# JohannesErnst/WeaSAL

Hardware: AMD Instinct MI355X
Metric: points/sec fwd+bwd KPFCNN on DALES spheres; achieved HBM GB/s on KPConv gather (higher is better)
Workload: dtype f32; 1 GPU; DALES_PseudoLabel KP-FCNN, in_radius=10m, 50k pts/sphere, batch=8, fp32, step = GPU pyramid + fwd + loss + bwd + SGD; contrast_loss term included (trainer_PseudoLabel.py:204-208); pyramid of the next batch overlapped on a second stream; parallelism=dp1, dist_world_size=1, allreduce_bytes=0

## Files before the change

include/weasal_hip.h:

```cpp
#ifndef WEASAL_HIP_H
#define WEASAL_HIP_H

#include <stdint.h>

#ifdef __cplusplus
extern "C" {
#endif

typedef enum {
    WS_OK = 0,
    WS_ERR_INVALID = 1,
    WS_ERR_UNSUPPORTED = 2,
    WS_ERR_HIP = 3,
    WS_ERR_EMPTY = 4,
    WS_ERR_CAPACITY = 5
} ws_status;

enum { WS_INFLUENCE_LINEAR = 0, WS_INFLUENCE_CONSTANT = 1, WS_INFLUENCE_GAUSSIAN = 2 };
enum { WS_AGGREGATION_SUM = 0, WS_AGGREGATION_CLOSEST = 1 };

const char* ws_last_error(void);
int64_t ws_launch_count(void);
const char* ws_version(void);
int ws_device_count(void);
// ... 96 lines not shown
                                     int32_t* d_max_count, void* stream);
int ws_radius_neighbors_nearest_async(ws_neighbors_ws* ws, const float* queries, int64_t nq, const float* supports,
                                      int64_t ns, const int32_t* h_q_lens, const int32_t* h_s_lens, int32_t nb,
                                      float radius, int32_t* out_i32, int64_t* out_i64, int32_t* d_any, void* stream);
int ws_radius_neighbors_order(const ws_neighbors_ws* ws, int32_t* out_order, void* stream);
const int32_t* ws_radius_neighbors_counts(const ws_neighbors_ws* ws);

int ws_radius_neighbors_set_key_last(ws_neighbors_ws* ws, uint64_t* d_key_last);
int ws_radius_neighbors_reuse_grid(ws_neighbors_ws* ws, int32_t on);
int ws_radius_neighbors_grid_info(const ws_neighbors_ws* ws, int32_t* nb, int64_t* cells, int64_t* ns, int64_t* blob_bytes);
int ws_radius_neighbors_grid_export(const ws_neighbors_ws* ws, void* blob, void* stream);
int ws_kpconv_gather_bwd_x_grid(const float* s_pts, int64_t ns, const void* grid_blob, int32_t nb, int64_t cells,
                                const uint64_t* key_last, float radius, const float* dwf, int32_t ci,
                                const float* kernel_points, int32_t k, const float* deformed_kp, const float* modulations,
                                float extent, int32_t influence, int32_t aggregation, const int32_t* order, float* dx,
                                int32_t* overflow, void* stream);

int ws_kpconv_gather_bwd_x_gated(const float* q_pts, int64_t nq, const float* s_pts, int64_t ns,
                                 const int64_t* inds, int32_t h, const int32_t* t_offsets, const int32_t* t_pairs,
                                 const float* dwf, int32_t ci, const float* kernel_points, int32_t k,
                                 const float* deformed_kp, const float* modulations, float extent,
                                 int32_t influence, int32_t aggregation, const int32_t* order, const float* gate_y,
                                 float gate_slope, float* dx, void* stream);
int ws_kpconv_gather_bwd_x_grid_gated(const float* s_pts, int64_t ns, const void* grid_blob, int32_t nb, int64_t cells,
                                      const uint64_t* key_last, float radius, const float* dwf, int32_t ci,
                                      const float* kernel_points, int32_t k, const float* deformed_kp, const float* modulations,
                                      float extent, int32_t influence, int32_t aggregation, const int32_t* order,
                                      const float* gate_y, float gate_slope, const int64_t* rows, int32_t rows_h, float* dx,
                                      int32_t* overflow, void* stream);

enum { WS_ORDER_REFERENCE = 0, WS_ORDER_FIRST_SEEN = 1 };
typedef struct ws_subsample_ws ws_subsample_ws;
int ws_subsample_ws_create(ws_subsample_ws** ws);
void ws_subsample_ws_destroy(ws_subsample_ws* ws);
int ws_grid_subsample_plan(ws_subsample_ws* ws, const float* points, int64_t n,
                           const int32_t* h_lens, int32_t nb, float dl, int32_t max_p,
                           int32_t order_mode, int32_t* h_out_lens, int64_t* h_m, void* stream);
int ws_grid_subsample_fill(ws_subsample_ws* ws,
                           const float* features, int32_t fd,
                           const int32_t* labels, int32_t ld,
                           float* out_points, float* out_features, int32_t* out_labels,
                           uint64_t* out_keys,
                           int32_t* out_counts,
                           void* stream);

int ws_rotate_clouds(const float* points, int64_t n, const int32_t* lens , int32_t nb,
// ... 304 lines not shown
```

weasal_amd/_lib.py:

```python
import ctypes as C
import os

_HERE = os.path.dirname(os.path.abspath(__file__))
LIB_PATH = os.path.join(_HERE, "libweasal_hip.so")

_vp = C.c_void_p
_i32 = C.c_int32
_i64 = C.c_int64
_f32 = C.c_float

SIGNATURES = {
    "ws_last_error": (C.c_char_p, []),
    "ws_version": (C.c_char_p, []),
    "ws_device_count": (C.c_int, []),
    "ws_kpconv_gather_fwd": (C.c_int, [_vp, _i64, _vp, _i64, _vp, _i32, _vp, _i32, _vp, _i32, _vp, _vp,
                                      _f32, _i32, _i32, _vp, _vp, _vp, _vp]),
    "ws_kpconv_gather_bwd_x": (C.c_int, [_vp, _i64, _vp, _i64, _vp, _i32, _vp, _vp, _vp, _i32, _vp, _i32,
                                        _vp, _vp, _f32, _i32, _i32, _vp, _vp, _vp]),
    "ws_kpconv_gather_bwd_geom": (C.c_int, [_vp, _i64, _vp, _i64, _vp, _i32, _vp, _i32, _vp, _vp, _i32,
                                           _vp, _vp, _vp, _f32, _i32, _i32, _vp, _vp, _vp]),
    "ws_transpose_scratch_bytes": (_i64, [_i64, _i32, _i64]),
    "ws_transpose_build": (C.c_int, [_vp, _i64, _i32, _i64, _vp, _vp, _vp, _vp]),
    "ws_max_pool_fwd": (C.c_int, [_vp, _i64, _i32, _vp, _i64, _i32, _vp, _vp, _vp]),
    "ws_max_pool_bwd": (C.c_int, [_vp, _vp, _i64, _i32, _i32, _vp, _vp, _i64, _vp, _vp]),
# ... 67 lines not shown
                                                   C.c_float, _i32, _i32, _vp, _vp, _vp, _vp]),
    "ws_max_pool_fwd_bf16": (C.c_int, [_vp, _i64, _i32, _vp, _i64, _i32, _vp, _vp, _vp]),
    "ws_max_pool_bwd_bf16": (C.c_int, [_vp, _vp, _i64, _i32, _i32, _vp, _vp, _i64, _vp, _vp]),
    "ws_closest_pool_fwd_bf16": (C.c_int, [_vp, _i64, _i32, _vp, _i64, _i32, _vp, _vp]),
    "ws_closest_pool_bwd_bf16": (C.c_int, [_vp, _i64, _i32, _i32, _vp, _vp, _i64, _vp, _vp]),
    "ws_gemm_xbt_bf16": (C.c_int, [_vp, _i64, _i32, _i64, _vp, _i32, _i64, _vp, _vp, _i64, _i32, _f32, _vp, _i64, _i32, _vp]),
    "ws_gemm_xty_bf16": (C.c_int, [_vp, _i64, _i32, _i64, _vp, _i32, _i64, _vp, _vp, _vp]),
    "ws_act_bwd_colsum_bf16_scratch_bytes": (_i64, [_i64, _i32]),
    "ws_act_bwd_colsum_bf16": (C.c_int, [_vp, _i32, _i64, _i32, _i64, _vp, _i64, C.c_float, _vp, _i64, _vp, _vp, _vp]),
    "ws_kpblock_fwd_scratch_bytes": (_i64, [_vp]),
    "ws_kpblock_bwd_scratch_bytes": (_i64, [_vp]),
    "ws_kpblock_fwd": (C.c_int, [_vp, _vp, _i64, _vp]),
    "ws_kpblock_bwd": (C.c_int, [_vp, _vp, _i64, _vp]),
    "ws_upunary_fwd_scratch_bytes": (_i64, [_vp]),
    "ws_upunary_bwd_scratch_bytes": (_i64, [_vp]),
    "ws_upunary_fwd": (C.c_int, [_vp, _vp, _i64, _vp]),
    "ws_upunary_bwd": (C.c_int, [_vp, _vp, _i64, _vp]),
    "ws_gemm_xb_epilogue_strided": (C.c_int, [_vp, _i64, _i32, _i64, _vp, _i64, _i64, _i32, _vp, _vp, _i64, _i32, _f32, _vp, _i64,
                                              _vp, _i64, _vp]),
    "ws_gemm_xb_gated_strided": (C.c_int, [_vp, _i64, _i32, _i64, _vp, _i64, _i64, _i32, _vp, _vp, _i64, _i32, _f32, _vp, _i64, _f32,
                                           _vp, _i64, _f32, _vp, _i64, _vp, _i64, _vp]),
    "ws_kpconv_gather_bwd_x_gated": (C.c_int, [_vp, _i64, _vp, _i64, _vp, _i32, _vp, _vp, _vp, _i32, _vp, _i32,
                                              _vp, _vp, _f32, _i32, _i32, _vp, _vp, _f32, _vp, _vp]),
    "ws_kpconv_gather_bwd_x_grid_gated": (C.c_int, [_vp, _i64, _vp, _i32, _i64, _vp, C.c_float, _vp, _i32, _vp, _i32, _vp, _vp,
                                                    C.c_float, _i32, _i32, _vp, _vp, _f32, _vp, _i32, _vp, _vp, _vp]),
    "ws_vote_update": (C.c_int, [_vp, _i64, _i32, _vp, _f32, _vp, _vp, _i64, _f32, _vp]),
    "ws_project_confusion": (C.c_int, [_vp, _i32, _vp, _i64, _vp, _vp, _i32, _vp, _vp]),
    "ws_potentials_scratch_bytes": (_i64, [_i64]),
    "ws_potentials_update": (C.c_int, [_vp, _i64, _vp, C.c_double, _vp, _vp, _vp, _vp, _vp]),
    "ws_al_point_scores": (C.c_int, [_vp, _i64, _i32, _vp, _vp, _vp, _vp, _vp]),
    "ws_al_anchor_scores": (C.c_int, [_vp, _vp, _i64, _vp, _vp, _i64, _i64, _vp, _i32, _vp, _vp]),
    "ws_topk_scratch_bytes": (_i64, [_i64, _i64]),
    "ws_topk_select": (C.c_int, [_vp, _i64, _vp, _i64, _i64, _vp, _vp, _vp]),
    "ws_weak_mask": (C.c_int, [_vp, _i64, _i32, _vp, _vp, _i64, _vp, _i64, _vp, _i64, _vp, _vp]),
    "ws_refine_labels": (C.c_int, [_vp, _vp, _i64, _i32, _vp, _vp, _i64, C.c_double, _i32, _vp, _vp, _i32, _vp, _vp]),
    "ws_anchor_bounds": (C.c_int, [_vp, _i64, _vp, _vp]),
    "ws_anchor_scratch_bytes": (_i64, [_i64]),
    "ws_anchor_members_plan": (C.c_int, [_vp, _vp, _i64, _i32, _vp, _i64, C.c_double, _vp, _vp, _vp, _vp, _vp, _vp, _vp, _vp, _vp,
                                        _vp, _vp]),
    "ws_anchor_members_fill": (C.c_int, [_vp, _i64, _vp, _i64, C.c_double, _vp, _vp, _vp, _vp, _vp, _vp, _vp, _i64, _i64, _vp, _vp,
                                        _vp, _vp, _vp, _vp, _vp]),
    "ws_anchor_pairs_plan": (C.c_int, [_vp, _i64, _vp, _i64, C.c_double, _vp, _vp, _vp, _vp, _vp, _vp, _vp, _vp, _vp]),
    "ws_anchor_pairs_fill": (C.c_int, [_vp, _i64, _vp, _i64, C.c_double, _vp, _vp, _vp, _vp, _i64, _vp, _vp, _vp]),
    "ws_anchor_overlap_plan": (C.c_int, [_vp, _vp, _i64, _vp, _i64, _vp, _i64, _vp, _vp, _i64, _vp, _vp, _vp, _vp, _vp, _vp, _vp]),
    "ws_anchor_overlap_fill": (C.c_int, [_vp, _i64, _vp, _vp, _i64, _vp, _vp, _i64, _vp, _i64, _vp, _vp, _i64, _vp, _vp, _vp, _vp,
                                        _i64, _i64, _i64, _vp, _vp, _vp, _vp, _vp]),
# ... 99 lines not shown
```

weasal_amd/csrc/blocks.hip:

```cpp
#include <vector>

#include "ws_common.h"

extern "C" int ws_block_gates = 1;
extern "C" int ws_block_gather_residual = 1;
extern "C" int64_t ws_block_group_rows = (int64_t)1 << 62;
extern "C" int ws_block_fused_infer = 1;
extern "C" int ws_block_pool_order = 1;

namespace {

struct Arena {
    char* base;
    int64_t cap, off;
    Arena(void* b, int64_t c) : base((char*)b), cap(c), off(0) {}
    template <typename T> T* take(int64_t count)
    {
        off = (off + 255) & ~(int64_t)255;
        T* p = base ? reinterpret_cast<T*>(base + off) : nullptr;
        off += count * (int64_t)sizeof(T);
        return p;
    }
    bool fits() const { return off <= cap; }
};

inline int64_t arena_bytes(const Arena& ar) { return ((ar.off + 255) & ~(int64_t)255) + 256; }

inline int64_t max3(int64_t a, int64_t b, int64_t c) { return a > b ? (a > c ? a : c) : (b > c ? b : c); }

__global__ __launch_bounds__(256) void transpose_small_kernel(const float* __restrict__ w, int rows, int cols, int64_t ld,
                                                               float* __restrict__ out)
// ... 300 lines not shown
                                            tmp_bytes, st));
        gin = g2;
        yconv = d->x2;
    }
    if (!d->w2 && d->dout_pregated) {
        if (d->dbk) WS_TRY(ws_act_bwd_colsum(gin, nq, d->conv_out, d->conv_out, nullptr, 0, 0.0f, nullptr, 0, d->dbk, tmp, st));
        g2 = const_cast<float*>(gin);
    } else if (!gated2)
        WS_TRY(ws_act_bwd_colsum(gin, nq, d->conv_out, d->conv_out, yconv, d->conv_out, d->slope, g2, d->conv_out, d->dbk, tmp, st));
    WS_TRY(leaves.add(d->wf, nq, kc, kc, g2, d->conv_out, d->conv_out, d->dwk, 0, t_dwk, b_dwk));
    if (!need_dx1) return leaves.flush();
    WS_TRY(linear_fwd(lk, g2, nq, d->conv_out, nullptr, nullptr, 0, 0, 0.0f, dwf, trk, tmp, tmp_bytes, st));
    float* dx1_out = d->w1 ? dx1 : d->dfeat;
    const float* gate1 = (d->w1 && !d->db1 && ws_block_gates) ? d->x1 : nullptr;
    if (!d->w1 && d->gate_dfeat && d->dfeat) gate1 = d->feat;
    if (d->grid_blob) {
        WS_REQUIRE(d->key_last && d->grid_overflow && nq == ns, "grid backward needs key_last / overflow and a self-query layer");
        WS_TRY(ws_kpconv_gather_bwd_x_grid_gated(d->s_pts, ns, d->grid_blob, d->grid_nb, d->grid_cells, d->key_last, d->grid_radius, dwf,
                                                 d->conv_in, d->kernel_points, d->k, nullptr, nullptr, d->extent, WS_INFLUENCE_LINEAR,
                                                 WS_AGGREGATION_SUM, d->order_s, gate1, d->slope, d->inds, d->h, dx1_out,
                                                 d->grid_overflow, st));
    } else {
        WS_REQUIRE(d->t_offsets && d->t_pairs, "KPConv backward needs the search grid or the transposed table");
        WS_TRY(ws_kpconv_gather_bwd_x_gated(d->q_pts, nq, d->s_pts, ns, d->inds, d->h, d->t_offsets, d->t_pairs, dwf, d->conv_in,
                                            d->kernel_points, d->k, nullptr, nullptr, d->extent, WS_INFLUENCE_LINEAR,
                                            WS_AGGREGATION_SUM, d->order_s, gate1, d->slope, dx1_out, st));
    }
    if (d->w1) {
        if (!gate1)
            WS_TRY(ws_act_bwd_colsum(dx1, ns, d->conv_in, d->conv_in, d->x1, d->conv_in, d->slope, dx1, d->conv_in, d->db1, tmp, st));
        WS_TRY(leaves.add(dx1, ns, d->conv_in, d->conv_in, d->feat, d->in_dim, d->in_dim, d->dw1, 0, t_dw1, b_dw1));
        if (d->dfeat)
            WS_TRY(ws_gemm_xb_gated_strided(dx1, ns, d->conv_in, d->conv_in, d->w1, d->in_dim, 1, d->in_dim, nullptr, sc_res, d->in_dim,
                                            0, 0.0f, d->gate_dfeat ? d->feat : nullptr, d->in_dim, d->slope, nullptr, 0, 0.0f, d->dfeat,
                                            d->in_dim, tmp, tmp_bytes, st));
    } else if (d->dfeat && sc_res) {
        WS_REQUIRE(!d->gate_dfeat, "gate_dfeat: a block without unary1 has no shortcut to add after the gate");
        const int64_t n4 = ns * d->in_dim / 4;
        add_rows_kernel<<<ws_grid(n4, 256), 256, 0, st>>>(d->dfeat, sc_res, n4);
        WS_LAUNCH_CHECK();
    }
    if (d->dfeat && d->dfeat_add && !added) {
        WS_REQUIRE(d->in_dim % 4 == 0, "dfeat_add needs in_dim %% 4 == 0");
        const int64_t n4 = ns * d->in_dim / 4;
        add_rows_kernel<<<ws_grid(n4, 256), 256, 0, st>>>(d->dfeat, d->dfeat_add, n4);
        WS_LAUNCH_CHECK();
    }
    return leaves.flush();
}
// ... 197 lines not shown
```

weasal_amd/csrc/kpconv.hip:

```cpp
#include "ws_common.h"
#include <algorithm>
#include "ws_grid.h"
#include "ws_bf16.h"

namespace {

constexpr float WS_SHADOW = 1e6f;

struct GeomParams {
    float extent;
    int influence;
    int aggregation;
    int deformable;
    const void* gate;
    float gate_slope;
    const int64_t* rows;
    int rows_h;
    const float4* kp4;
    const float* rmax;
    int cut;
    int ilv;
    int csplit;
};

// ... 851 lines not shown
                            const float md = modulations[q * K + k];
#pragma unroll
                            for (int t = 0; t < NT; ++t) v[t] *= md;
                        }
                        RowLoad<NT, T>::st(wf + (q * K + k) * ci + ch, v);
                    }
                }
            }
        }
        if (DEF && min_d2) {
            mind = fminf(mind, __shfl_xor(mind, 16, 64));
            mind = fminf(mind, __shfl_xor(mind, 32, 64));
            if (kk == 0 && haskp) min_d2[q * K + i] = mind;
        }
        p0x = idx1 >= 0 ? p1x : WS_SHADOW; p0y = idx1 >= 0 ? p1y : WS_SHADOW; p0z = idx1 >= 0 ? p1z : WS_SHADOW;
        idx0 = idx1;
        idx1 = chk(raw2);
        qv0 = qv1; qv1 = qv2; qv2 = qv3;
        qx = q1x; qy = q1y; qz = q1z;
        q1x = q2x; q1y = q2y; q1z = q2z;
    }
}

template <int K, int G, int MODE, bool VEC, typename T = float>
__global__ __launch_bounds__(256) void kpconv_gather_bwd_x_kernel(
    const float* __restrict__ q_pts, int64_t nq, const float* __restrict__ s_pts, int64_t ns,
    int h, const int32_t* __restrict__ t_offsets, const int32_t* __restrict__ t_pairs,
    const T* __restrict__ dwf, int ci, const float* __restrict__ kernel_points,
    const float* __restrict__ deformed_kp, const float* __restrict__ modulations, GeomParams g,
    T* __restrict__ dx, const int32_t* __restrict__ order)
{
    constexpr int CC = 4 * G;
    constexpr int S = 64 / G;
    static_assert(K <= 16 && POOL >= 16 * K, "pool sizing");
    __shared__ uint2 pool_all[4][POOL_ALLOC];
    __shared__ int segs_all[4][K + 1];
    const int wave = __builtin_amdgcn_readfirstlane(threadIdx.x >> 6);
    const int lane = threadIdx.x & 63;
    uint2* pool = pool_all[wave];
    int* segs = segs_all[wave];
    const int j = lane % G;
    const int slot = lane / G;
    const float inv_extent = 1.0f / g.extent;

    float kpr[MODE == 0 ? 3 * K : 1];
    if (MODE == 0) {
#pragma unroll
        for (int t = 0; t < 3 * K; ++t) kpr[t] = kernel_points[t];
    }

    int64_t item0, istep, iend;
    ws_wave_items(ns, order ? g.ilv : 0, wave, item0, istep, iend);
    for (int64_t item = item0; item < iend; item += istep) {
        const int64_t s = order ? (int64_t)order[item] : item;
        const float sx = s_pts[3 * s + 0], sy = s_pts[3 * s + 1], sz = s_pts[3 * s + 2];
        const int beg = t_offsets[s], end = t_offsets[s + 1];
        for (int cc0 = 0; cc0 < ci; cc0 += CC) {
            float4 acc = make_float4(0.f, 0.f, 0.f, 0.f);
            const int ch = cc0 + 4 * j;
            const bool chok = VEC ? (ch + 3 < ci) : (ch < ci);
            const int chl = chok ? ch : 0;
            float4 gq = make_float4(1.f, 1.f, 1.f, 1.f);
            if (g.gate && slot == 0) {
                const T* gy = reinterpret_cast<const T*>(g.gate) + s * ci + ch;
                if (VEC) {
                    if (chok) gq = ld4(gy);
                } else {
                    if (ch + 0 < ci) gq.x = ld1(gy + 0);
                    if (ch + 1 < ci) gq.y = ld1(gy + 1);
                    if (ch + 2 < ci) gq.z = ld1(gy + 2);
                    if (ch + 3 < ci) gq.w = ld1(gy + 3);
                }
            }
            auto flush = [&](int total) {
                wave_lds_sync();
                total = min(total, POOL);
                const int per = (total + S - 1) / S;
// ... 72 lines not shown
                acc.y += __shfl_xor(acc.y, o, 64);
                acc.z += __shfl_xor(acc.z, o, 64);
                acc.w += __shfl_xor(acc.w, o, 64);
            }
            if (slot == 0) {
                T* dst = dx + s * ci + ch;
                if (g.gate) {
                    acc.x *= gq.x > 0.0f ? 1.0f : g.gate_slope; acc.y *= gq.y > 0.0f ? 1.0f : g.gate_slope;
                    acc.z *= gq.z > 0.0f ? 1.0f : g.gate_slope; acc.w *= gq.w > 0.0f ? 1.0f : g.gate_slope;
                }
                if (VEC) {
                    if (chok) st4(dst, acc);
                } else {
                    if (ch + 0 < ci) st1(dst + 0, acc.x);
                    if (ch + 1 < ci) st1(dst + 1, acc.y);
                    if (ch + 2 < ci) st1(dst + 2, acc.z);
                    if (ch + 3 < ci) st1(dst + 3, acc.w);
                }
            }
        }
    }
}

template <int K, typename T = float>
__global__ __launch_bounds__(256) void kpconv_gather_bwd_geom_kernel(
    const float* __restrict__ q_pts, int64_t nq, const float* __restrict__ s_pts, int64_t ns,
    const int64_t* __restrict__ inds, int h, const T* __restrict__ x, int ci,
    const T* __restrict__ dwf, const float* __restrict__ deformed_kp,
    const float* __restrict__ modulations, const float* __restrict__ d_min_d2, GeomParams g,
    float* __restrict__ d_kp, float* __restrict__ d_mod, int vec4)
{
    const int wave = __builtin_amdgcn_readfirstlane(threadIdx.x >> 6);
    const int lane = threadIdx.x & 63;
    for (int64_t q = (int64_t)blockIdx.x * 4 + wave; q < nq; q += (int64_t)gridDim.x * 4) {
        const float qx = q_pts[3 * q + 0], qy = q_pts[3 * q + 1], qz = q_pts[3 * q + 2];
        const float* kp = deformed_kp + q * (3 * K);
        float gk[K][3];
        float gm[K];
        float best[K];
        int bestcol[K];
#pragma unroll
        for (int k = 0; k < K; ++k) {
            gk[k][0] = gk[k][1] = gk[k][2] = 0.0f;
            gm[k] = 0.0f;
            best[k] = 3.4e38f;
            bestcol[k] = 0x7fffffff;
// ... 772 lines not shown
                        if (ch + 0 < ci) st1(dst + 0, a.x);
                        if (ch + 1 < ci) st1(dst + 1, a.y);
                        if (ch + 2 < ci) st1(dst + 2, a.z);
                        if (ch + 3 < ci) st1(dst + 3, a.w);
                    }
                }
            }
            wave_lds_order();
        }
    }
}

}

extern "C" int ws_kpconv_grid_sorted;
int ws_kpconv_grid_sorted = 0;

#include <cstdio>
#include <type_traits>

namespace {

constexpr int SPLIT_ROWS = 4096;
constexpr int SPLIT_NT = 4;
constexpr int GRID_INTERLEAVE = 512;

enum { GK_FWD_MFMA, GK_FWD_POOL, GK_BWD_X, GK_BWD_GEOM, GK_BWD_X_GRID, GK_BWD_X_GRIDW, GK_BWD_GEOM_DEF };
struct GatherPlan {
    int kernel;
    bool bf16;
    int n;
    int mode;
    bool def;
    bool vec;
    int pw;
    bool cut;
    int nch;
    bool sort;
    bool areg;
    int grid;
    int csplit, ilv, rows_sorted;
};

int nt_for_rows(int ci, const void* a, const void* b)
{
    const int nt = ci <= 16 ? 1 : (ci <= 32 ? 2 : (ci <= 64 ? 4 : (ci <= 128 ? 8 : 16)));
    return (ci % nt == 0 && (nt == 1 || (aligned16(a) && aligned16(b)))) ? nt : 1;
}
int group_ladder(int ci) { return ci <= 4 ? 1 : (ci <= 8 ? 2 : (ci <= 16 ? 4 : (ci <= 32 ? 8 : 16))); }
bool rows_vec4(bool bf16, int ci, const void* a, const void* b)
// ... 43 lines not shown
        return WS_OK;
    }
    p.mode = (!deformed && influence == WS_INFLUENCE_LINEAR && aggregation == WS_AGGREGATION_SUM) ? 0 : 1;
    p.n = p.vec ? 1 : 4; p.pw = p.vec ? 4 : 1;
    return WS_OK;
}

int fwd_def_plan(bool bf16, int64_t nq, int32_t ci, const void* x, const void* wf, bool rows_sorted, GatherPlan& p)
{
    p = new_plan(GK_FWD_MFMA, bf16, nq);
    p.n = nt_for_rows(ci, x, wf);
    p.mode = 2; p.def = true; p.vec = true; p.cut = rows_sorted;
    if (bf16 && p.n == 1 && (ci % 2)) return ws_fail(WS_ERR_UNSUPPORTED, "bf16 rows need an even channel count (ci=%d)", ci);
    return WS_OK;
}

int bwd_x_plan(bool bf16, int64_t ns, int32_t ci, const void* dwf, const void* dx, int mode, GatherPlan& p)
{
    p = new_plan(GK_BWD_X, bf16, ns);
    p.n = group_ladder(ci); p.mode = mode;
    return rows_vec4_or_f32(bf16, ci, dwf, dx, p.vec);
}

int bwd_geom_plan(bool bf16, int64_t nq, int32_t ci, const void* x, const void* dwf, GatherPlan& p)
{
    p = new_plan(GK_BWD_GEOM, bf16, nq);
    p.mode = 1; p.vec = rows_vec4(bf16, ci, x, dwf);
    return WS_OK;
}

int bwd_x_grid_plan(bool bf16, int64_t ns, int32_t ci, const void* dwf, const void* dx, int mode, bool ordered, GatherPlan& p)
{
    p = new_plan(GK_BWD_X_GRID, bf16, ns);
    p.n = group_ladder(ci); p.mode = mode; p.sort = ws_kpconv_grid_sorted != 0;
    grid_walk_plan(ns, ordered, p);
    return rows_vec4_or_f32(bf16, ci, dwf, dx, p.vec);
}

int bwd_x_gridw_plan(bool bf16, int64_t ns, int32_t ci, const void* dwf, const void* dx, bool deformed, bool ordered, GatherPlan& p)
{
    p = new_plan(GK_BWD_X_GRIDW, bf16, ns);
    p.n = group_ladder(ci); p.mode = deformed ? 2 : 0;
    p.nch = (p.n < 16 || ci <= 64) ? 1 : (ci <= 128 ? 2 : 4);
    grid_walk_plan(ns, ordered, p);
    return rows_vec4_or_f32(bf16, ci, dwf, dx, p.vec);
}
// ... 5 lines not shown
        return ws_fail(WS_ERR_UNSUPPORTED, "geometry backward on the matrix core needs ci %% 16 == 0 and 16-byte aligned rows (ci=%d)", ci);
    p.mode = 2; p.vec = true; p.cut = rows_sorted;
    p.areg = ci == 16 || ci == 32 || ci == 64 || ci == 128;
    p.n = p.areg ? ci / 4 : (ci % 128 == 0 ? 32 : (ci % 64 == 0 ? 16 : (ci % 32 == 0 ? 8 : 4)));
    return WS_OK;
}

void plan_text(const GatherPlan& p, char* out, size_t n)
{
    const char* t = p.bf16 ? "bf16" : "float";
    auto b = [](bool v) { return v ? "true" : "false"; };
    switch (p.kernel) {
    case GK_FWD_MFMA:
        snprintf(out, n, "kpconv_gather_fwd_mfma_kernel<NT=%d, MODE=%d, DEF=%s, VECROW=%s, T=%s, CUT=%s> grid=%d csplit=%d", p.n, p.mode,
                 b(p.def), b(p.vec), t, b(p.cut), p.grid, p.csplit);
        break;
    case GK_FWD_POOL:
        snprintf(out, n, "kpconv_gather_fwd_kernel<K=15, G=%d, MODE=%d, DEF=%s, VEC=%s, PW=%d, T=%s> grid=%d csplit=%d cut=%d", p.n, p.mode,
                 b(p.def), b(p.vec), p.pw, t, p.grid, p.csplit, p.rows_sorted);
        break;
    case GK_BWD_X:
        snprintf(out, n, "kpconv_gather_bwd_x_kernel<K=15, G=%d, MODE=%d, VEC=%s, T=%s> grid=%d", p.n, p.mode, b(p.vec), t, p.grid);
        break;
    case GK_BWD_GEOM:
        snprintf(out, n, "kpconv_gather_bwd_geom_kernel<K=15, T=%s> grid=%d vec4=%d", t, p.grid, p.vec ? 1 : 0);
        break;
    case GK_BWD_X_GRID:
        snprintf(out, n, "kpconv_gather_bwd_x_grid_kernel<K=15, G=%d, MODE=%d, VEC=%s, T=%s, SORT=%s> grid=%d ilv=%d", p.n, p.mode, b(p.vec),
                 t, b(p.sort), p.grid, p.ilv);
        break;
    case GK_BWD_X_GRIDW:
        snprintf(out, n, "kpconv_gather_bwd_x_gridw_kernel<K=15, G=%d, MODE=%d, VEC=%s, NCH=%d, T=%s> grid=%d ilv=%d", p.n, p.mode,
                 b(p.vec), p.nch, t, p.grid, p.ilv);
        break;
    default:
        snprintf(out, n, "kpconv_gather_bwd_geom_def_kernel<CK=%d, AREG=%s, T=%s, CUT=%s> grid=%d", p.n, b(p.areg), t, b(p.cut), p.grid);
    }
}

template <int... Vs> struct Pick { int v; };
using Flag = Pick<0, 1>;
template <typename F> void dispatch(F&& f) { f(); }
template <typename F, int... Vs, typename... Rest>
void dispatch(F&& f, Pick<Vs...> a, Rest... rest)
{
    (void)(((a.v == Vs) && (dispatch([&](auto... cs) { f(std::integral_constant<int, Vs>{}, cs...); }, rest...), true)) || ...);
// ... 20 lines not shown
                     int32_t h, const void* x, int32_t ci, const float* kernel_points, const float* deformed_kp, const float* modulations,
                     const GeomParams& g, void* wf, float* min_d2, const int32_t* order)
{
    dispatch([&](auto bf, auto nt, auto mode, auto def, auto cut) {
        using T = Row<bf.value>;
        if constexpr (mode.value == 1 ? !cut.value : def.value == (mode.value == 2))
            kpconv_gather_fwd_mfma_kernel<nt.value, mode.value, def.value != 0, true, T, 0, cut.value != 0><<<p.grid, 256, 0, (hipStream_t)stream>>>(
                q_pts, nq, s_pts, ns, inds, h, (const T*)x, ci, kernel_points, deformed_kp, modulations, g, (T*)wf, min_d2, order);
    }, Flag{p.bf16}, Pick<1, 2, 4, 8, 16>{p.n}, Pick<0, 1, 2>{p.mode}, Flag{p.def}, Flag{p.cut});
}

void launch_bwd_x(const GatherPlan& p, void* stream, const float* q_pts, int64_t nq, const float* s_pts, int64_t ns, int32_t h,
                  const int32_t* t_offsets, const int32_t* t_pairs, const void* dwf, int32_t ci, const float* kernel_points,
                  const float* deformed_kp, const float* modulations, const GeomParams& g, void* dx, const int32_t* order)
{
    dispatch([&](auto bf, auto gr, auto mode, auto vec) {
        using T = Row<bf.value>;
        if constexpr (!bf.value || vec.value)
            kpconv_gather_bwd_x_kernel<15, gr.value, mode.value, vec.value != 0, T><<<p.grid, 256, 0, (hipStream_t)stream>>>(
                q_pts, nq, s_pts, ns, h, t_offsets, t_pairs, (const T*)dwf, ci, kernel_points, deformed_kp, modulations, g, (T*)dx, order);
    }, Flag{p.bf16}, Pick<1, 2, 4, 8, 16>{p.n}, Pick<0, 1, 2>{p.mode}, Flag{p.vec});
}

int gather_bwd_x_impl(bool bf16, const float* q_pts, int64_t nq, const float* s_pts, int64_t ns, int32_t h, const int32_t* t_offsets,
                      const int32_t* t_pairs, const void* dwf, int32_t ci, const float* kernel_points, int32_t k, const float* deformed_kp,
                      const float* modulations, float extent, int32_t influence, int32_t aggregation, const int32_t* order, void* dx,
                      void* stream, const void* gate = nullptr, float gate_slope = 0.0f)
{
    if (int rc = check_common(q_pts, nq, s_pts, ns, h, ci, k, extent, influence, aggregation)) return rc;
    if (ns == 0) return WS_OK;
    WS_REQUIRE(t_offsets && t_pairs && dwf && dx && (kernel_points || deformed_kp), "NULL argument");
    WS_REQUIRE(nq * (int64_t)h < (1ll << 31), "nq*h exceeds int32");
    WS_REQUIRE(nq * (int64_t)k * ci < (1ll << 31), "nq*k*ci exceeds the 32-bit row offsets of the gather");
    GatherPlan p;
    if (int rc = bwd_x_plan(bf16, ns, ci, dwf, dx, rigid_fast(deformed_kp, modulations, influence, aggregation) ? 0 : 1, p)) return rc;
    GeomParams g{extent, influence, aggregation, deformed_kp ? 1 : 0, gate, gate_slope, nullptr, 0};
    launch_bwd_x(p, stream, q_pts, nq, s_pts, ns, h, t_offsets, t_pairs, dwf, ci, kernel_points, deformed_kp, modulations, g, dx, order);
    return launched();
}

int gather_bwd_geom_impl(bool bf16, const float* q_pts, int64_t nq, const float* s_pts, int64_t ns, const int64_t* inds, int32_t h,
                         const void* x, int32_t ci, const void* dwf, int32_t k, const float* deformed_kp, const float* modulations,
                         const float* d_min_d2, float extent, int32_t influence, int32_t aggregation, float* d_deformed_kp,
                         float* d_modulations, void* stream)
{
    if (int rc = check_common(q_pts, nq, s_pts, ns, h, ci, k, extent, influence, aggregation)) return rc;
    if (nq == 0) return WS_OK;
    WS_REQUIRE(inds && x && dwf && deformed_kp && d_deformed_kp, "NULL argument");
    GatherPlan p;
    if (int rc = bwd_geom_plan(bf16, nq, ci, x, dwf, p)) return rc;
    GeomParams g{extent, influence, aggregation, 1, nullptr, 0.0f, nullptr, 0};
    dispatch([&](auto bf) {
        using T = Row<bf.value>;
        kpconv_gather_bwd_geom_kernel<15, T><<<p.grid, 256, 0, (hipStream_t)stream>>>(
            q_pts, nq, s_pts, ns, inds, h, (const T*)x, ci, (const T*)dwf, deformed_kp, modulations, d_min_d2, g, d_deformed_kp, d_modulations,
            p.vec);
    }, Flag{p.bf16});
    return launched();
}
// ... 272 lines not shown
}

int ws_kpconv_gather_bwd_x_grid_bf16(const float* s_pts, int64_t ns, const void* grid_blob, int32_t nb, int64_t cells,
                                     const uint64_t* key_last, float radius, const uint16_t* dwf, int32_t ci,
                                     const float* kernel_points, int32_t k, const float* deformed_kp, const float* modulations,
                                     float extent, int32_t influence, int32_t aggregation, const int32_t* order, uint16_t* dx,
                                     int32_t* overflow, void* stream)
{
    return gather_bwd_x_grid_impl(true, s_pts, ns, grid_blob, nb, cells, key_last, radius, dwf, ci, kernel_points, k, deformed_kp,
                                  modulations, extent, influence, aggregation, order, dx, overflow, stream);
}

int ws_kpconv_gather_bwd_x_gated(const float* q_pts, int64_t nq, const float* s_pts, int64_t ns,
                                 const int64_t* inds, int32_t h, const int32_t* t_offsets, const int32_t* t_pairs,
                                 const float* dwf, int32_t ci, const float* kernel_points, int32_t k,
                                 const float* deformed_kp, const float* modulations, float extent,
                                 int32_t influence, int32_t aggregation, const int32_t* order, const float* gate_y,
                                 float gate_slope, float* dx, void* stream)
{
    return gather_bwd_x_impl(false, q_pts, nq, s_pts, ns, h, t_offsets, t_pairs, dwf, ci, kernel_points, k, deformed_kp, modulations, extent,
                             influence, aggregation, order, dx, stream, gate_y, gate_slope);
}

int ws_kpconv_gather_bwd_x_grid_gated(const float* s_pts, int64_t ns, const void* grid_blob, int32_t nb, int64_t cells,
                                      const uint64_t* key_last, float radius, const float* dwf, int32_t ci,
                                      const float* kernel_points, int32_t k, const float* deformed_kp, const float* modulations,
                                      float extent, int32_t influence, int32_t aggregation, const int32_t* order,
                                      const float* gate_y, float gate_slope, const int64_t* rows, int32_t rows_h, float* dx,
                                      int32_t* overflow, void* stream)
{
    return gather_bwd_x_grid_impl(false, s_pts, ns, grid_blob, nb, cells, key_last, radius, dwf, ci, kernel_points, k, deformed_kp,
                                  modulations, extent, influence, aggregation, order, dx, overflow, stream, gate_y, gate_slope, rows, rows_h);
}

}
```

weasal_amd/fused.py:

```python
import ctypes as C
import os
import weakref

import torch

from . import _lib, ops
from ._lib import check, current_stream

FUSED_BLOCKS = os.environ.get("WEASAL_FUSED_BLOCKS", "1") != "0"
FUSED_INFER = os.environ.get("WEASAL_FUSED_INFER", "1") != "0"
_timed = False


_timed_min_rows = 0


def set_timed(on, min_rows=0):
    global _timed, _timed_min_rows
    _timed = bool(on)
    _timed_min_rows = int(min_rows)


_vp, _i32, _i64, _f32 = C.c_void_p, C.c_int32, C.c_int64, C.c_float

# ... 11 lines not shown
                ("db2", _vp), ("dws", _vp), ("timed", _i32), ("rows_sorted", _i32), ("infer", _i32), ("dout_pregated", _i32),
                ("gate_dfeat", _i32), ("dfeat_add", _vp)]


class UpUnaryDesc(C.Structure):
    _fields_ = [("xc", _vp), ("nc", _i64), ("c_up", _i32), ("skip", _vp), ("nf", _i64), ("c_skip", _i32),
                ("ups", _vp), ("h_up", _i32), ("t_offsets", _vp), ("t_pairs", _vp),
                ("w", _vp), ("ldw", _i64), ("b", _vp), ("out_dim", _i32), ("relu", _i32), ("slope", _f32),
                ("yc", _vp), ("out", _vp), ("dout", _vp), ("dxc", _vp), ("dskip", _vp), ("dw", _vp), ("db", _vp),
                ("drop_p", _f32), ("drop_seed", C.c_uint64), ("dout_pregated", _i32), ("gate_dxc", _i32)]


_GATES_SET = False


def _bind():
    global _GATES_SET
    lib = _lib.lib()
    if not _GATES_SET:
        C.c_int.in_dll(lib, "ws_block_gates").value = 0 if os.environ.get("WEASAL_BLOCK_GATES", "1") == "0" else 1
        C.c_int.in_dll(lib, "ws_block_fused_infer").value = 1 if FUSED_INFER else 0
        C.c_int.in_dll(lib, "ws_block_gather_residual").value = 0 if os.environ.get("WEASAL_BLOCK_GATHER_RESIDUAL", "1") == "0" else 1
        C.c_int.in_dll(lib, "ws_block_pool_order").value = 0 if os.environ.get("WEASAL_POOL_ORDER", "1") == "0" else 1
        if "WEASAL_BLOCK_GROUP_ROWS" in os.environ:
            C.c_int64.in_dll(lib, "ws_block_group_rows").value = int(os.environ["WEASAL_BLOCK_GROUP_ROWS"])
        _GATES_SET = True
    return lib


def timer_records(layer=False):
    lib = _bind()
    out = []
    nq, h, ci, ms, ml = _i64(), _i32(), _i32(), _f32(), _f32()
    for i in range(lib.ws_timer_count()):
        check(lib.ws_timer_read(i, C.byref(nq), C.byref(h), C.byref(ci), C.byref(ms)))
        if layer:
            check(lib.ws_timer_read_layer(i, C.byref(ml)))
            out.append((nq.value, h.value, ci.value, ms.value, ml.value))
        else:
            out.append((nq.value, h.value, ci.value, ms.value))
    return out


def timer_reset():
    _bind().ws_timer_reset()

# ... 368 lines not shown
```

Baseline: 32.15 million points/s.

## Add packed KPConv backward-x kernel handling four supports per wave

Adds a packed backward-x gather kernel that assigns one support point to each 16-lane group, so a wave handles four supports at once. Kernel-point weights are built with ballot/popcount into per-group LDS pools, and supports with more than 16 neighbours or too many nonzero weights fall back to the existing per-support routine. The point is to stop wasting a full 64-lane wave on supports with few neighbours (the nq<ns pooling/strided case). It costs extra divergence and a fallback path, and it only engages for rigid fp32 vec4 layers with a low mean neighbour count. Enabled by default through a block flag.

```diff
diff --git a/include/weasal_hip.h b/include/weasal_hip.h
--- a/include/weasal_hip.h
+++ b/include/weasal_hip.h
@@ -142,6 +142,15 @@
                                  const float* deformed_kp, const float* modulations, float extent,
                                  int32_t influence, int32_t aggregation, const int32_t* order, const float* gate_y,
                                  float gate_slope, float* dx, void* stream);
+int ws_kpconv_gather_bwd_x_packed(const float* q_pts, int64_t nq, const float* s_pts, int64_t ns,
+                                  const int64_t* inds, int32_t h, const int32_t* t_offsets, const int32_t* t_pairs,
+                                  const float* dwf, int32_t ci, const float* kernel_points, int32_t k,
+                                  const float* deformed_kp, const float* modulations, float extent,
+                                  int32_t influence, int32_t aggregation, const int32_t* order, const float* gate_y,
+                                  float gate_slope, float* dx, void* stream);
+int ws_kpconv_gather_bwd_x_packed_variant(int64_t nq, int64_t ns, int32_t h, int32_t ci, const void* dwf, const void* dx, int32_t deformed,
+                                          int32_t modulated, int32_t influence, int32_t aggregation, int32_t rows_bf16, int32_t ordered,
+                                          char* out, int32_t cap);
 int ws_kpconv_gather_bwd_x_grid_gated(const float* s_pts, int64_t ns, const void* grid_blob, int32_t nb, int64_t cells,
                                       const uint64_t* key_last, float radius, const float* dwf, int32_t ci,
                                       const float* kernel_points, int32_t k, const float* deformed_kp, const float* modulations,
diff --git a/weasal_amd/_lib.py b/weasal_amd/_lib.py
--- a/weasal_amd/_lib.py
+++ b/weasal_amd/_lib.py
@@ -113,6 +113,10 @@
                                            _vp, _i64, _f32, _vp, _i64, _vp, _i64, _vp]),
     "ws_kpconv_gather_bwd_x_gated": (C.c_int, [_vp, _i64, _vp, _i64, _vp, _i32, _vp, _vp, _vp, _i32, _vp, _i32,
                                               _vp, _vp, _f32, _i32, _i32, _vp, _vp, _f32, _vp, _vp]),
+    "ws_kpconv_gather_bwd_x_packed": (C.c_int, [_vp, _i64, _vp, _i64, _vp, _i32, _vp, _vp, _vp, _i32, _vp, _i32,
+                                               _vp, _vp, _f32, _i32, _i32, _vp, _vp, _f32, _vp, _vp]),
+    "ws_kpconv_gather_bwd_x_packed_variant": (C.c_int, [_i64, _i64, _i32, _i32, _vp, _vp, _i32, _i32, _i32, _i32, _i32, _i32,
+                                                       C.c_char_p, _i32]),
     "ws_kpconv_gather_bwd_x_grid_gated": (C.c_int, [_vp, _i64, _vp, _i32, _i64, _vp, C.c_float, _vp, _i32, _vp, _i32, _vp, _vp,
                                                     C.c_float, _i32, _i32, _vp, _vp, _f32, _vp, _i32, _vp, _vp, _vp]),
     "ws_vote_update": (C.c_int, [_vp, _i64, _i32, _vp, _f32, _vp, _vp, _i64, _f32, _vp]),
diff --git a/weasal_amd/csrc/blocks.hip b/weasal_amd/csrc/blocks.hip
--- a/weasal_amd/csrc/blocks.hip
+++ b/weasal_amd/csrc/blocks.hip
@@ -7,6 +7,7 @@
 extern "C" int64_t ws_block_group_rows = (int64_t)1 << 62;
 extern "C" int ws_block_fused_infer = 1;
 extern "C" int ws_block_pool_order = 1;
+extern "C" int ws_block_packed_k4 = 1;
 
 namespace {
 
@@ -353,9 +354,9 @@
                                                  d->grid_overflow, st));
     } else {
         WS_REQUIRE(d->t_offsets && d->t_pairs, "KPConv backward needs the search grid or the transposed table");
-        WS_TRY(ws_kpconv_gather_bwd_x_gated(d->q_pts, nq, d->s_pts, ns, d->inds, d->h, d->t_offsets, d->t_pairs, dwf, d->conv_in,
-                                            d->kernel_points, d->k, nullptr, nullptr, d->extent, WS_INFLUENCE_LINEAR,
-                                            WS_AGGREGATION_SUM, d->order_s, gate1, d->slope, dx1_out, st));
+        WS_TRY((ws_block_packed_k4 ? ws_kpconv_gather_bwd_x_packed : ws_kpconv_gather_bwd_x_gated)(
+            d->q_pts, nq, d->s_pts, ns, d->inds, d->h, d->t_offsets, d->t_pairs, dwf, d->conv_in, d->kernel_points, d->k, nullptr, nullptr,
+            d->extent, WS_INFLUENCE_LINEAR, WS_AGGREGATION_SUM, d->order_s, gate1, d->slope, dx1_out, st));
     }
     if (d->w1) {
         if (!gate1)
diff --git a/weasal_amd/csrc/kpconv.hip b/weasal_amd/csrc/kpconv.hip
--- a/weasal_amd/csrc/kpconv.hip
+++ b/weasal_amd/csrc/kpconv.hip
@@ -897,37 +897,18 @@
     }
 }
 
-template <int K, int G, int MODE, bool VEC, typename T = float>
-__global__ __launch_bounds__(256) void kpconv_gather_bwd_x_kernel(
-    const float* __restrict__ q_pts, int64_t nq, const float* __restrict__ s_pts, int64_t ns,
-    int h, const int32_t* __restrict__ t_offsets, const int32_t* __restrict__ t_pairs,
-    const T* __restrict__ dwf, int ci, const float* __restrict__ kernel_points,
-    const float* __restrict__ deformed_kp, const float* __restrict__ modulations, GeomParams g,
-    T* __restrict__ dx, const int32_t* __restrict__ order)
+template <int K, int G, int MODE, bool VEC, typename T>
+__device__ __forceinline__ void bwd_x_support(
+    int64_t s, const float* __restrict__ q_pts, const float* __restrict__ s_pts, int h, const int32_t* __restrict__ t_offsets,
+    const int32_t* __restrict__ t_pairs, const T* __restrict__ dwf, int ci, const float* __restrict__ kernel_points,
+    const float* __restrict__ deformed_kp, const float* __restrict__ modulations, const GeomParams& g, T* __restrict__ dx,
+    const float (&kpr)[MODE == 0 ? 3 * K : 1], float inv_extent, uint2* pool, int* segs, int lane)
 {
     constexpr int CC = 4 * G;
     constexpr int S = 64 / G;
-    static_assert(K <= 16 && POOL >= 16 * K, "pool sizing");
-    __shared__ uint2 pool_all[4][POOL_ALLOC];
-    __shared__ int segs_all[4][K + 1];
-    const int wave = __builtin_amdgcn_readfirstlane(threadIdx.x >> 6);
-    const int lane = threadIdx.x & 63;
-    uint2* pool = pool_all[wave];
-    int* segs = segs_all[wave];
     const int j = lane % G;
     const int slot = lane / G;
-    const float inv_extent = 1.0f / g.extent;
-
-    float kpr[MODE == 0 ? 3 * K : 1];
-    if (MODE == 0) {
-#pragma unroll
-        for (int t = 0; t < 3 * K; ++t) kpr[t] = kernel_points[t];
-    }
-
-    int64_t item0, istep, iend;
-    ws_wave_items(ns, order ? g.ilv : 0, wave, item0, istep, iend);
-    for (int64_t item = item0; item < iend; item += istep) {
-        const int64_t s = order ? (int64_t)order[item] : item;
+    {
         const float sx = s_pts[3 * s + 0], sy = s_pts[3 * s + 1], sz = s_pts[3 * s + 2];
         const int beg = t_offsets[s], end = t_offsets[s + 1];
         for (int cc0 = 0; cc0 < ci; cc0 += CC) {
@@ -1046,6 +1027,186 @@
     }
 }
 
+template <int K, int G, int MODE, bool VEC, typename T = float>
+__global__ __launch_bounds__(256) void kpconv_gather_bwd_x_kernel(
+    const float* __restrict__ q_pts, int64_t nq, const float* __restrict__ s_pts, int64_t ns,
+    int h, const int32_t* __restrict__ t_offsets, const int32_t* __restrict__ t_pairs,
+    const T* __restrict__ dwf, int ci, const float* __restrict__ kernel_points,
+    const float* __restrict__ deformed_kp, const float* __restrict__ modulations, GeomParams g,
+    T* __restrict__ dx, const int32_t* __restrict__ order)
+{
+    static_assert(K <= 16 && POOL >= 16 * K, "pool sizing");
+    __shared__ uint2 pool_all[4][POOL_ALLOC];
+    __shared__ int segs_all[4][K + 1];
+    const int wave = __builtin_amdgcn_readfirstlane(threadIdx.x >> 6);
+    const int lane = threadIdx.x & 63;
+    uint2* pool = pool_all[wave];
+    int* segs = segs_all[wave];
+    const float inv_extent = 1.0f / g.extent;
+
+    float kpr[MODE == 0 ? 3 * K : 1];
+    if (MODE == 0) {
+#pragma unroll
+        for (int t = 0; t < 3 * K; ++t) kpr[t] = kernel_points[t];
+    }
+
+    int64_t item0, istep, iend;
+    ws_wave_items(ns, order ? g.ilv : 0, wave, item0, istep, iend);
+    for (int64_t item = item0; item < iend; item += istep) {
+        const int64_t s = order ? (int64_t)order[item] : item;
+        bwd_x_support<K, G, MODE, VEC, T>(s, q_pts, s_pts, h, t_offsets, t_pairs, dwf, ci, kernel_points, deformed_kp, modulations, g, dx,
+                                          kpr, inv_extent, pool, segs, lane);
+    }
+}
+
+template <int K, int G, bool VEC, typename T = float>
+__global__ __launch_bounds__(256) void kpconv_gather_bwd_x_packed_kernel(
+    const float* __restrict__ q_pts, int64_t nq, const float* __restrict__ s_pts, int64_t ns,
+    int h, const int32_t* __restrict__ t_offsets, const int32_t* __restrict__ t_pairs,
+    const T* __restrict__ dwf, int ci, const float* __restrict__ kernel_points,
+    const float* __restrict__ deformed_kp, const float* __restrict__ modulations, GeomParams g,
+    T* __restrict__ dx, const int32_t* __restrict__ order)
+{
+    constexpr int CC = 4 * G;
+    constexpr int S = 64 / G;
+    constexpr int QP = POOL / 4;
+    static_assert(VEC && G <= 16 && K <= 16 && POOL >= 16 * K, "float4 rows, a support per 16 lanes");
+    __shared__ uint2 pool_all[4][POOL_ALLOC];
+    __shared__ int segs_all[4][K + 1];
+    const int wave = __builtin_amdgcn_readfirstlane(threadIdx.x >> 6);
+    const int lane = threadIdx.x & 63;
+    uint2* pool = pool_all[wave];
+    const int grp = lane >> 4, li = lane & 15;
+    const int j = li % G;
+    const int rslot = li / G;
+    const unsigned gbase = (unsigned)(grp * QP), dummy = (unsigned)(POOL + 8 + lane);
+    const unsigned below = (1u << li) - 1u;
+    const float inv_extent = 1.0f / g.extent;
+
+    float kpr[3 * K];
+#pragma unroll
+    for (int t = 0; t < 3 * K; ++t) kpr[t] = kernel_points[t];
+
+    int64_t ibeg, iend;
+    ws_block_range(ns, ibeg, iend);
+    for (int64_t item = ibeg + 4 * wave; item < iend; item += 16) {
+        const int64_t mine = item + grp;
+        const bool have = mine < iend;
+        const int64_t s = have ? (order ? (int64_t)order[mine] : mine) : 0;
+        const int beg = have ? t_offsets[s] : 0, end = have ? t_offsets[s + 1] : 0;
+        const bool fits16 = have && end - beg <= 16;
+        const bool real = fits16 && beg + li < end;
+        const int pair = real ? t_pairs[beg + li] : 0;
+        const int q = pair / h;
+        float nx = 0.f, ny = 0.f, nz = 0.f;
+        if (real) {
+            nx = s_pts[3 * s + 0] - q_pts[3 * (int64_t)q + 0];
+            ny = s_pts[3 * s + 1] - q_pts[3 * (int64_t)q + 1];
+            nz = s_pts[3 * s + 2] - q_pts[3 * (int64_t)q + 2];
+        }
+        int total = 0;
+#pragma unroll
+        for (int k = 0; k < K; ++k) {
+            const float ex = nx - kpr[3 * k + 0], ey = ny - kpr[3 * k + 1], ez = nz - kpr[3 * k + 2];
+            const float d = (ex * ex + ey * ey) + ez * ez;
+            float w = fmaxf(1.0f - __builtin_amdgcn_sqrtf(d) * inv_extent, 0.0f);
+            w = real ? w : 0.0f;
+            const unsigned long long m = __ballot(w != 0.0f);
+            const unsigned half = grp >= 2 ? (unsigned)(m >> 32) : (unsigned)m;
+            const unsigned gm = (half >> (16 * (grp & 1))) & 0xffffu;
+            const unsigned pos = (unsigned)total + (unsigned)__builtin_popcount(gm & below);
+            const bool ok = (w != 0.0f) && pos < (unsigned)QP;
+            pool[ok ? gbase + pos : dummy] = make_uint2((unsigned)(q * K + k), __float_as_uint(w));
+            total += __builtin_popcount(gm);
+        }
+        const bool packed = fits16 && total <= QP;
+        const unsigned long long single = __ballot(have && !packed && li == 0);
+        total = packed ? total : 0;
+        wave_lds_sync();
+        const int per = (total + S - 1) / S;
+        for (int cc0 = 0; cc0 < ci; cc0 += CC) {
+            const int ch = cc0 + 4 * j;
+            const bool chok = ch + 3 < ci;
+            const int chl = chok ? ch : 0;
+            float4 gq = make_float4(1.f, 1.f, 1.f, 1.f);
+            if (g.gate && rslot == 0 && packed && chok) gq = ld4(reinterpret_cast<const T*>(g.gate) + s * ci + ch);
+            float4 pad = make_float4(0.f, 0.f, 0.f, 0.f);
+            if (per & 3) pad = load_row_piece<VEC>(dwf, 0u, ci, chl);
+            float4 a[4];
+            int lo[4], hi[4];
+#pragma unroll
+            for (int u = 0; u < 4; ++u) {
+                a[u] = make_float4(0.f, 0.f, 0.f, 0.f);
+                lo[u] = (4 * rslot + u) * per;
+                hi[u] = chok ? min(lo[u] + per, total) : lo[u];
+            }
+            for (int it = 0; it < per; ++it) {
+                float4 v[4];
+                float w[4];
+                uint2 e[4];
+#pragma unroll
+                for (int u = 0; u < 4; ++u) {
+                    e[u] = pool[gbase + (unsigned)min(lo[u] + it, QP - 1)];
+                    keep_unconditional(e[u]);
+                }
+#pragma unroll
+                for (int u = 0; u < 4; ++u) {
+                    const bool ok = lo[u] + it < hi[u];
+                    e[u].x = ok ? e[u].x : 0u;
+                    w[u] = ok ? __uint_as_float(e[u].y) : 0.0f;
+                    v[u] = load_row_piece<VEC>(dwf, e[u].x, ci, chl);
+                }
+#pragma unroll
+                for (int u = 0; u < 4; ++u) {
+                    a[u].x = fmaf(w[u], v[u].x, a[u].x);
+                    a[u].y = fmaf(w[u], v[u].y, a[u].y);
+                    a[u].z = fmaf(w[u], v[u].z, a[u].z);
+                    a[u].w = fmaf(w[u], v[u].w, a[u].w);
+                }
+            }
+            if (per & 3) {
+#pragma unroll
+                for (int u = 0; u < 4; ++u) {
+                    a[u].x = fmaf(0.0f, pad.x, a[u].x);
+                    a[u].y = fmaf(0.0f, pad.y, a[u].y);
+                    a[u].z = fmaf(0.0f, pad.z, a[u].z);
+                    a[u].w = fmaf(0.0f, pad.w, a[u].w);
+                }
+            }
+            float4 acc;
+            acc.x = (a[0].x + a[1].x) + (a[2].x + a[3].x);
+            acc.y = (a[0].y + a[1].y) + (a[2].y + a[3].y);
+            acc.z = (a[0].z + a[1].z) + (a[2].z + a[3].z);
+            acc.w = (a[0].w + a[1].w) + (a[2].w + a[3].w);
+#pragma unroll
+            for (int o = G; o < 16; o <<= 1) {
+                acc.x += __shfl_xor(acc.x, o, 64);
+                acc.y += __shfl_xor(acc.y, o, 64);
+                acc.z += __shfl_xor(acc.z, o, 64);
+                acc.w += __shfl_xor(acc.w, o, 64);
+            }
+            if (rslot == 0 && packed && chok) {
+                if (g.gate) {
+                    acc.x *= gq.x > 0.0f ? 1.0f : g.gate_slope; acc.y *= gq.y > 0.0f ? 1.0f : g.gate_slope;
+                    acc.z *= gq.z > 0.0f ? 1.0f : g.gate_slope; acc.w *= gq.w > 0.0f ? 1.0f : g.gate_slope;
+                }
+                st4(dx + s * ci + ch, acc);
+            }
+        }
+        wave_lds_sync();
+        if (single) {
+#pragma unroll 1
+            for (int t = 0; t < 4; ++t) {
+                if ((single >> (16 * t)) & 1ull) {
+                    const int64_t s1 = order ? (int64_t)order[item + t] : item + t;
+                    bwd_x_support<K, G, 0, VEC, T>(s1, q_pts, s_pts, h, t_offsets, t_pairs, dwf, ci, kernel_points, nullptr, nullptr, g, dx,
+                                                   kpr, inv_extent, pool, segs_all[wave], lane);
+                }
+            }
+        }
+    }
+}
+
 template <int K, typename T = float>
 __global__ __launch_bounds__(256) void kpconv_gather_bwd_geom_kernel(
     const float* __restrict__ q_pts, int64_t nq, const float* __restrict__ s_pts, int64_t ns,
@@ -1864,10 +2025,11 @@
 namespace {
 
 constexpr int SPLIT_ROWS = 4096;
+constexpr int PACK_MEAN_MAX = 12;
 constexpr int SPLIT_NT = 4;
 constexpr int GRID_INTERLEAVE = 512;
 
-enum { GK_FWD_MFMA, GK_FWD_POOL, GK_BWD_X, GK_BWD_GEOM, GK_BWD_X_GRID, GK_BWD_X_GRIDW, GK_BWD_GEOM_DEF };
+enum { GK_FWD_MFMA, GK_FWD_POOL, GK_BWD_X, GK_BWD_GEOM, GK_BWD_X_GRID, GK_BWD_X_GRIDW, GK_BWD_GEOM_DEF, GK_BWD_X_PACKED };
 struct GatherPlan {
     int kernel;
     bool bf16;
@@ -1957,6 +2119,17 @@
     return rows_vec4_or_f32(bf16, ci, dwf, dx, p.vec);
 }
 
+int bwd_x_packed_plan(bool bf16, int64_t nq, int64_t ns, int32_t h, int32_t ci, const void* dwf, const void* dx, int mode, bool ordered,
+                      GatherPlan& p)
+{
+    if (int rc = bwd_x_plan(bf16, ns, ci, dwf, dx, mode, p)) return rc;
+    (void)ordered;
+    if (bf16 || !p.vec || mode != 0 || nq >= ns || nq * (int64_t)h > (int64_t)PACK_MEAN_MAX * ns) return WS_OK;
+    p.kernel = GK_BWD_X_PACKED;
+    p.grid = ws_grid(ws_ceil_div(ns, 4), 4);
+    return WS_OK;
+}
+
 int bwd_geom_plan(bool bf16, int64_t nq, int32_t ci, const void* x, const void* dwf, GatherPlan& p)
 {
     p = new_plan(GK_BWD_GEOM, bf16, nq);
@@ -2008,6 +2181,9 @@
     case GK_BWD_X:
         snprintf(out, n, "kpconv_gather_bwd_x_kernel<K=15, G=%d, MODE=%d, VEC=%s, T=%s> grid=%d", p.n, p.mode, b(p.vec), t, p.grid);
         break;
+    case GK_BWD_X_PACKED:
+        snprintf(out, n, "kpconv_gather_bwd_x_packed_kernel<K=15, G=%d, VEC=%s, T=%s> grid=%d", p.n, b(p.vec), t, p.grid);
+        break;
     case GK_BWD_GEOM:
         snprintf(out, n, "kpconv_gather_bwd_geom_kernel<K=15, T=%s> grid=%d vec4=%d", t, p.grid, p.vec ? 1 : 0);
         break;
@@ -2074,10 +2250,20 @@
     }, Flag{p.bf16}, Pick<1, 2, 4, 8, 16>{p.n}, Pick<0, 1, 2>{p.mode}, Flag{p.vec});
 }
 
+void launch_bwd_x_packed(const GatherPlan& p, void* stream, const float* q_pts, int64_t nq, const float* s_pts, int64_t ns, int32_t h,
+                         const int32_t* t_offsets, const int32_t* t_pairs, const float* dwf, int32_t ci, const float* kernel_points,
+                         const GeomParams& g, float* dx, const int32_t* order)
+{
+    dispatch([&](auto gr) {
+        kpconv_gather_bwd_x_packed_kernel<15, gr.value, true, float><<<p.grid, 256, 0, (hipStream_t)stream>>>(
+            q_pts, nq, s_pts, ns, h, t_offsets, t_pairs, dwf, ci, kernel_points, nullptr, nullptr, g, dx, order);
+    }, Pick<1, 2, 4, 8, 16>{p.n});
+}
+
 int gather_bwd_x_impl(bool bf16, const float* q_pts, int64_t nq, const float* s_pts, int64_t ns, int32_t h, const int32_t* t_offsets,
                       const int32_t* t_pairs, const void* dwf, int32_t ci, const float* kernel_points, int32_t k, const float* deformed_kp,
                       const float* modulations, float extent, int32_t influence, int32_t aggregation, const int32_t* order, void* dx,
-                      void* stream, const void* gate = nullptr, float gate_slope = 0.0f)
+                      void* stream, const void* gate = nullptr, float gate_slope = 0.0f, bool packed = false)
 {
     if (int rc = check_common(q_pts, nq, s_pts, ns, h, ci, k, extent, influence, aggregation)) return rc;
     if (ns == 0) return WS_OK;
@@ -2085,8 +2271,14 @@
     WS_REQUIRE(nq * (int64_t)h < (1ll << 31), "nq*h exceeds int32");
     WS_REQUIRE(nq * (int64_t)k * ci < (1ll << 31), "nq*k*ci exceeds the 32-bit row offsets of the gather");
     GatherPlan p;
-    if (int rc = bwd_x_plan(bf16, ns, ci, dwf, dx, rigid_fast(deformed_kp, modulations, influence, aggregation) ? 0 : 1, p)) return rc;
+    const int mode = rigid_fast(deformed_kp, modulations, influence, aggregation) ? 0 : 1;
+    if (int rc = packed ? bwd_x_packed_plan(bf16, nq, ns, h, ci, dwf, dx, mode, order != nullptr, p) : bwd_x_plan(bf16, ns, ci, dwf, dx, mode, p))
+        return rc;
     GeomParams g{extent, influence, aggregation, deformed_kp ? 1 : 0, gate, gate_slope, nullptr, 0};
+    if (p.kernel == GK_BWD_X_PACKED) {
+        launch_bwd_x_packed(p, stream, q_pts, nq, s_pts, ns, h, t_offsets, t_pairs, (const float*)dwf, ci, kernel_points, g, (float*)dx, order);
+        return launched();
+    }
     launch_bwd_x(p, stream, q_pts, nq, s_pts, ns, h, t_offsets, t_pairs, dwf, ci, kernel_points, deformed_kp, modulations, g, dx, order);
     return launched();
 }
@@ -2405,6 +2597,30 @@
                              influence, aggregation, order, dx, stream, gate_y, gate_slope);
 }
 
+int ws_kpconv_gather_bwd_x_packed(const float* q_pts, int64_t nq, const float* s_pts, int64_t ns,
+                                  const int64_t* inds, int32_t h, const int32_t* t_offsets, const int32_t* t_pairs,
+                                  const float* dwf, int32_t ci, const float* kernel_points, int32_t k,
+                                  const float* deformed_kp, const float* modulations, float extent,
+                                  int32_t influence, int32_t aggregation, const int32_t* order, const float* gate_y,
+                                  float gate_slope, float* dx, void* stream)
+{
+    return gather_bwd_x_impl(false, q_pts, nq, s_pts, ns, h, t_offsets, t_pairs, dwf, ci, kernel_points, k, deformed_kp, modulations, extent,
+                             influence, aggregation, order, dx, stream, gate_y, gate_slope, true);
+}
+
+int ws_kpconv_gather_bwd_x_packed_variant(int64_t nq, int64_t ns, int32_t h, int32_t ci, const void* dwf, const void* dx, int32_t deformed,
+                                          int32_t modulated, int32_t influence, int32_t aggregation, int32_t rows_bf16, int32_t ordered,
+                                          char* out, int32_t cap)
+{
+    WS_REQUIRE(out && cap > 0 && ci >= 1 && h >= 1 && nq >= 0 && ns >= 0, "bad argument");
+    GatherPlan p;
+    const int mode = rigid_fast(deformed != 0, modulated != 0, influence, aggregation) ? 0 : 1;
+    if (int rc = bwd_x_packed_plan(rows_bf16 != 0, nq, ns, h, ci, dwf, dx, mode, ordered != 0, p)) return rc;
+    if (p.kernel == GK_BWD_X_PACKED) plan_text(p, out, (size_t)cap);
+    else snprintf(out, (size_t)cap, "none");
+    return WS_OK;
+}
+
 int ws_kpconv_gather_bwd_x_grid_gated(const float* s_pts, int64_t ns, const void* grid_blob, int32_t nb, int64_t cells,
                                       const uint64_t* key_last, float radius, const float* dwf, int32_t ci,
                                       const float* kernel_points, int32_t k, const float* deformed_kp, const float* modulations,
diff --git a/weasal_amd/fused.py b/weasal_amd/fused.py
--- a/weasal_amd/fused.py
+++ b/weasal_amd/fused.py
@@ -57,6 +57,7 @@
         C.c_int.in_dll(lib, "ws_block_fused_infer").value = 1 if FUSED_INFER else 0
         C.c_int.in_dll(lib, "ws_block_gather_residual").value = 0 if os.environ.get("WEASAL_BLOCK_GATHER_RESIDUAL", "1") == "0" else 1
         C.c_int.in_dll(lib, "ws_block_pool_order").value = 0 if os.environ.get("WEASAL_POOL_ORDER", "1") == "0" else 1
+        C.c_int.in_dll(lib, "ws_block_packed_k4").value = 0 if os.environ.get("WEASAL_BLOCK_PACKED_K4", "1") == "0" else 1
         if "WEASAL_BLOCK_GROUP_ROWS" in os.environ:
             C.c_int64.in_dll(lib, "ws_block_group_rows").value = int(os.environ["WEASAL_BLOCK_GROUP_ROWS"])
         _GATES_SET = True
```

After: 32.74 million points/s (median of 6 runs). 1.02x the previous value.
